# automl/CARL

Hardware: AMD Instinct MI355X
Metric: env-steps/sec (whole node) at 65k parallel contexts, 1/2/4/8 MI355X (higher is better)
Workload: dtype f32

## Files before the change

carl_amd/csrc/carl_policy.hip:

```cpp
#include <hip/hip_runtime.h>

#include <cstdint>

#include "../../include/carl_amd.h"
#include "classic_control.hip.h"
#include "host_common.hpp"
#include "policy_host.hpp"
#include "policy_kernels.hip.h"

namespace carl_host {

int policy_set_floats(const carl_policy_t* p) {
  if (p->n_in < 1 || p->n_in > CARL_POLICY_MAX_IN || p->n_out < 1 || p->n_out > 4 || p->n_hidden < 0 ||
      p->n_hidden > CARL_POLICY_MAX_HIDDEN)
    return -1;
  int64_t total = 0, prev = p->n_in;
  for (int l = 0; l <= p->n_hidden; ++l) {
    const int64_t w = l < p->n_hidden ? p->width[l] : p->n_out;
    if (l < p->n_hidden && (w < 1 || w > CARL_POLICY_MAX_WIDTH)) return -1;
    total += w * prev + w;
    prev = w;
  }
  total += 2 * (int64_t)p->n_in + 1;
  return (int)((total + 3) / 4 * 4);
}

int policy_padded_hidden(const carl_policy_t* p) {
  int wmax = 0;
  for (int l = 0; l < p->n_hidden; ++l) wmax = wmax > p->width[l] ? wmax : p->width[l];
  return p->n_hidden == 0 ? 0 : wmax <= 32 ? 32 : 64;
}

namespace {

int validate_policy(const carl_batch_t* b, const carl_policy_t* p, const carl_family_info_t& fi, const char* who) {
  if (p->n_hidden < 0 || p->n_hidden > CARL_POLICY_MAX_HIDDEN)
    return fail(CARL_ERR_INVALID_ARGUMENT, "%s: n_hidden %d outside [0, %d]", who, p->n_hidden, CARL_POLICY_MAX_HIDDEN);
  for (int l = 0; l < p->n_hidden; ++l)
    if (p->width[l] < 1 || p->width[l] > CARL_POLICY_MAX_WIDTH)
      return fail(CARL_ERR_INVALID_ARGUMENT, "%s: hidden width[%d] = %d outside [1, %d]", who, l, p->width[l],
                  CARL_POLICY_MAX_WIDTH);
  if (p->n_ctx < 0 || p->n_ctx > fi.n_features)
    return fail(CARL_ERR_INVALID_ARGUMENT, "%s: n_ctx %d outside [0, F = %d]", who, p->n_ctx, fi.n_features);
  for (int k = 0; k < p->n_ctx; ++k)
    if (p->ctx_rows[k] < 0 || p->ctx_rows[k] >= fi.n_features)
      return fail(CARL_ERR_INVALID_ARGUMENT, "%s: ctx_rows[%d] = %d is not a context-table row (F = %d)", who, k,
                  p->ctx_rows[k], fi.n_features);
  if (p->n_in != p->n_ctx + fi.obs_dim)
    return fail(CARL_ERR_INVALID_ARGUMENT, "%s: n_in %d != n_ctx %d + obs_dim %d", who, p->n_in, p->n_ctx, fi.obs_dim);
  const int want_out = fi.action_is_discrete ? fi.n_actions : 1;
  if (p->n_out != want_out)
    return fail(CARL_ERR_INVALID_ARGUMENT, "%s: head width %d, the family needs %d (%s)", who, p->n_out, want_out,
                fi.action_is_discrete ? "n_actions" : "one Box value");
  if (p->head != (fi.action_is_discrete ? CARL_POLICY_HEAD_ARGMAX : CARL_POLICY_HEAD_BOX))
    return fail(CARL_ERR_INVALID_ARGUMENT, "%s: head kind %d does not match the family's action space", who, p->head);
  if (p->activation < CARL_POLICY_IDENTITY || p->activation > CARL_POLICY_RELU)
    return fail(CARL_ERR_INVALID_ARGUMENT, "%s: unknown activation %d", who, p->activation);
  if (p->n_sets < 1) return fail(CARL_ERR_INVALID_ARGUMENT, "%s: n_sets %d < 1", who, p->n_sets);
  if (p->lanes_per_set < carl::kPolicyLanes || p->lanes_per_set % carl::kPolicyLanes != 0)
    return fail(CARL_ERR_INVALID_ARGUMENT, "%s: lanes_per_set %d is not a positive multiple of %d (carl_policy_lane_quantum)",
                who, p->lanes_per_set, carl::kPolicyLanes);
  if ((int64_t)p->n_sets * p->lanes_per_set < b->n_lanes)
    return fail(CARL_ERR_INVALID_ARGUMENT, "%s: %d sets x %d lanes do not cover %d lanes", who, p->n_sets,
                p->lanes_per_set, b->n_lanes);
  if (p->params == nullptr) return fail(CARL_ERR_INVALID_ARGUMENT, "%s: params is NULL", who);
  return 0;
}

int validate_io(const carl_batch_t* b, const carl_step_io_t* io, const carl_family_info_t& fi, const char* who) {
  if (!io->action || !io->obs || !io->reward || !io->terminated || !io->truncated)
    return fail(CARL_ERR_INVALID_ARGUMENT, "%s: a required io pointer is NULL", who);
  const int want = fi.action_is_discrete ? CARL_ACTION_I32 : CARL_ACTION_F32;
  if (io->action_dtype != want)
    return fail(CARL_ERR_INVALID_ARGUMENT, "%s: the action column is %s for this family", who,
                fi.action_is_discrete ? "int32 (CARL_ACTION_I32)" : "float32 (CARL_ACTION_F32)");
  if (io->row_pitch != 0 && io->row_pitch < b->n_lanes)
    return fail(CARL_ERR_INVALID_ARGUMENT, "%s: io.row_pitch %d < n_lanes %d", who, io->row_pitch, b->n_lanes);
  if (!carl_host::staged_rows(b, io, 15))
    return fail(CARL_ERR_UNSUPPORTED, "%s: rows of %d lanes for %d lanes: the closed-loop rollout writes the staged layout "
                "only (pitch %% 16 == 0 and n_lanes %% 16 == 0 or pitch == carl_rollout_pitch(n_lanes), arrays on 16-byte "
                "boundaries)", who, io->row_pitch > 0 ? io->row_pitch : b->n_lanes, b->n_lanes);
  return 0;
}

}

int check_rollout_policy(const char* who, const carl_batch_t* batch, const carl_policy_t* policy_host,
                         const carl_step_io_t* io, int32_t n_steps, const carl_policy_summary_t* summary_out,
                         carl_family_info_t* fi) {
  if (batch == nullptr || policy_host == nullptr) return fail(CARL_ERR_INVALID_ARGUMENT, "%s: batch / policy is NULL", who);
  if (batch->family >= CARL_N_FAMILIES)
    return fail(CARL_ERR_INVALID_ARGUMENT, "%s: family %d is a Brax family -- the closed-loop rollout covers the "
                "classic-control families only", who, batch->family);
  if (int e = validate_batch(batch, who)) return e;
  if (int e = carl_family_info(batch->family, fi)) return e;
  if (int e = validate_policy(batch, policy_host, *fi, who)) return e;
  if (n_steps < 0) return fail(CARL_ERR_INVALID_ARGUMENT, "%s: n_steps %d < 0", who, n_steps);
  if (io == nullptr) {
    if (summary_out == nullptr || !summary_out->episodes || !summary_out->return_sum || !summary_out->length_sum)
      return fail(CARL_ERR_INVALID_ARGUMENT, "%s: summary mode (io NULL) needs all three summary arrays", who);
  } else {
    if (int e = validate_io(batch, io, *fi, who)) return e;
    if (summary_out != nullptr && (!summary_out->episodes || !summary_out->return_sum || !summary_out->length_sum))
      return fail(CARL_ERR_INVALID_ARGUMENT, "%s: a summary needs all three arrays", who);
  }
  if (summary_out != nullptr && !(batch->flags & CARL_FLAG_AUTORESET))
    return fail(CARL_ERR_UNSUPPORTED, "%s: a summary needs CARL_FLAG_AUTORESET (without auto-reset a finished lane "
                "reports done on every later step, and its episode would be counted on each of them)", who);
  return 0;
}

int policy_rollout_without_steps(const char* who, const carl_batch_t* batch, const carl_policy_summary_t* summary_out,
                                 void* stream) {
  if (summary_out == nullptr || batch->n_lanes == 0) return 0;
  hipStream_t s = (hipStream_t)stream;
  const size_t bytes = (size_t)batch->n_lanes * 4;
  for (void* p : {(void*)summary_out->episodes, (void*)summary_out->return_sum, (void*)summary_out->length_sum})
    if (const hipError_t e = hipMemsetAsync(p, 0, bytes, s); e != hipSuccess)
      return fail((int)e, "%s: hipMemsetAsync: %s", who, hipGetErrorString(e));
  return 0;
}

int check_evaluate_policy(const char* who, const carl_batch_t* batch, const carl_policy_t* policy_host,
                          int32_t n_episodes, int32_t max_steps, const carl_policy_episodes_t* out,
                          carl_family_info_t* fi) {
  if (batch == nullptr || policy_host == nullptr)
    return fail(CARL_ERR_INVALID_ARGUMENT, "%s: batch / policy is NULL", who);
  if (batch->family >= CARL_N_FAMILIES)
    return fail(CARL_ERR_INVALID_ARGUMENT, "%s: family %d is a Brax family -- the closed-loop rollout covers the "
                "classic-control families only", who, batch->family);
  if (int e = validate_batch(batch, who)) return e;
  if (int e = carl_family_info(batch->family, fi)) return e;
  if (int e = validate_policy(batch, policy_host, *fi, who)) return e;
  if (out == nullptr || !out->episodes || !out->steps || !out->ret || !out->length || !out->context_id ||
      !out->terminated)
    return fail(CARL_ERR_INVALID_ARGUMENT, "%s: out and all six of its arrays are required", who);
  if (n_episodes < 1) return fail(CARL_ERR_INVALID_ARGUMENT, "%s: n_episodes %d < 1", who, n_episodes);
  if (max_steps < 0) return fail(CARL_ERR_INVALID_ARGUMENT, "%s: max_steps %d < 0", who, max_steps);
  if ((int64_t)n_episodes * batch->n_lanes >= ((int64_t)1 << 31))
    return fail(CARL_ERR_INVALID_ARGUMENT, "%s: n_episodes %d x %d lanes records do not fit 2^31 - 1", who, n_episodes,
                batch->n_lanes);
  if (!(batch->flags & CARL_FLAG_AUTORESET))
    return fail(CARL_ERR_UNSUPPORTED, "%s: needs CARL_FLAG_AUTORESET (without auto-reset a finished lane reports done on "
                "every later step, and its episode would be counted on each of them)", who);
  return 0;
}

}

namespace {

using carl_host::check_launch;
using carl_host::fail;

struct PolicyKernel {
  void (*fn)(carl_batch_t, carl_step_io_t, carl_policy_t, int, carl_policy_summary_t, int);
  size_t lds;
};

template <class Fam, int H>
PolicyKernel policy_kernel(bool summary) {
  if (summary) return {carl::policy_rollout_kernel<Fam, H, true>, carl::policy_lds_bytes<Fam, H, true>()};
  return {carl::policy_rollout_kernel<Fam, H, false>, carl::policy_lds_bytes<Fam, H, false>()};
}

template <class Fam>
int launch_policy(const carl_batch_t* b, const carl_policy_t* p, const carl_step_io_t* io, int n_steps,
                  const carl_policy_summary_t* sum, hipStream_t s) {
  const bool summary = io == nullptr;
  const int H = carl_host::policy_padded_hidden(p);
  const PolicyKernel k = H == 0 ? policy_kernel<Fam, 0>(summary) : H == 32 ? policy_kernel<Fam, 32>(summary)
                                                                  : policy_kernel<Fam, 64>(summary);
  static_assert(carl::policy_lds_bytes<Fam, 64, false>() + carl::static_lds_bytes<Fam>() <= carl::kCuLdsBytes,
                "the closed-loop rollout's LDS does not fit a compute unit");
  if (int e = carl_host::ensure_dynamic_lds(reinterpret_cast<const void*>(k.fn), k.lds, "carl_rollout_policy")) return e;
  carl_step_io_t io_r{};
  if (!summary) {
    io_r = *io;
    io_r.row_pitch = io->row_pitch > 0 ? io->row_pitch : b->n_lanes;
  }
  const carl_policy_summary_t sum_r = sum != nullptr ? *sum : carl_policy_summary_t{nullptr, nullptr, nullptr};
  const int grid = (b->n_lanes + carl::kPolicyLanes - 1) / carl::kPolicyLanes;
  const int threads = summary ? carl::kPolicyThreadsSummary : carl::kPolicyThreadsTransitions;
  hipLaunchKernelGGL(k.fn, dim3(grid), dim3(threads), k.lds, s, *b, io_r, *p, carl_host::policy_set_floats(p), sum_r, n_steps);
  return check_launch("carl_rollout_policy");
}

struct EpisodesKernel {
  void (*fn)(carl_batch_t, carl_policy_t, int, carl_policy_episodes_t, int, int);
  size_t lds;
};

template <class Fam, int H>
EpisodesKernel episodes_kernel() {
  return {carl::policy_episodes_kernel<Fam, H>, carl::policy_lds_bytes<Fam, H, true>()};
}

template <class Fam>
int launch_episodes(const carl_batch_t* b, const carl_policy_t* p, int n_episodes, int max_steps,
                    const carl_policy_episodes_t* out, hipStream_t s) {
  const int H = carl_host::policy_padded_hidden(p);
  const EpisodesKernel k = H == 0 ? episodes_kernel<Fam, 0>() : H == 32 ? episodes_kernel<Fam, 32>()
                                                               : episodes_kernel<Fam, 64>();
  if (int e = carl_host::ensure_dynamic_lds(reinterpret_cast<const void*>(k.fn), k.lds, "carl_evaluate_policy")) return e;
  const int grid = (b->n_lanes + carl::kPolicyLanes - 1) / carl::kPolicyLanes;
  hipLaunchKernelGGL(k.fn, dim3(grid), dim3(carl::kPolicyThreadsSummary), k.lds, s, *b, *p, carl_host::policy_set_floats(p), *out,
                     n_episodes, max_steps);
  return check_launch("carl_evaluate_policy");
}

}

extern "C" {

int32_t carl_policy_lane_quantum(void) { return carl::kPolicyLanes; }

int32_t carl_policy_set_floats(const carl_policy_t* policy_host) {
  if (policy_host == nullptr) return -1;
  return carl_host::policy_set_floats(policy_host);
}

int carl_rollout_policy(const carl_batch_t* batch, const carl_policy_t* policy_host, const carl_step_io_t* io,
                        int32_t n_steps, const carl_policy_summary_t* summary_out, void* stream) {
  const char* who = "carl_rollout_policy";
  carl_family_info_t fi;
  if (int e = carl_host::check_rollout_policy(who, batch, policy_host, io, n_steps, summary_out, &fi)) return e;
  if (batch->n_lanes == 0 || n_steps == 0) return carl_host::policy_rollout_without_steps(who, batch, summary_out, stream);
  return carl_host::with_classic_family(batch, [&](auto fam) {
    return launch_policy<decltype(fam)>(batch, policy_host, io, n_steps, summary_out, (hipStream_t)stream);
  });
}

int carl_evaluate_policy(const carl_batch_t* batch, const carl_policy_t* policy_host, int32_t n_episodes,
                         int32_t max_steps, const carl_policy_episodes_t* out, void* stream) {
  carl_family_info_t fi;
  if (int e = carl_host::check_evaluate_policy("carl_evaluate_policy", batch, policy_host, n_episodes, max_steps, out, &fi))
    return e;
  if (batch->n_lanes == 0) return 0;
  return carl_host::with_classic_family(batch, [&](auto fam) {
    return launch_episodes<decltype(fam)>(batch, policy_host, n_episodes, max_steps, out, (hipStream_t)stream);
  });
}

}
```

carl_amd/csrc/carl_policy_sample.hip:

```cpp
#include <hip/hip_runtime.h>

#include <cstdint>

#include "../../include/carl_amd.h"
#include "classic_control.hip.h"
#include "host_common.hpp"
#include "policy_host.hpp"
#include "policy_kernels.hip.h"

namespace {

using carl_host::check_launch;
using carl_host::fail;

int check_sampling(const char* who, const carl_policy_sampling_t* smp, const carl_family_info_t& fi, bool log_prob_ok) {
  if (smp == nullptr) return fail(CARL_ERR_INVALID_ARGUMENT, "%s: sampling is NULL", who);
  if (!fi.action_is_discrete && smp->log_std == nullptr)
    return fail(CARL_ERR_INVALID_ARGUMENT, "%s: a Box family needs sampling->log_std ([n_sets] on the device)", who);
  if (!log_prob_ok && smp->log_prob != nullptr)
    return fail(CARL_ERR_INVALID_ARGUMENT, "%s: sampling->log_prob is a transitions-mode output (io != NULL); this mode "
                "stores nothing per step", who);
  if ((reinterpret_cast<uintptr_t>(smp->log_prob) & 15) != 0)
    return fail(CARL_ERR_UNSUPPORTED, "%s: sampling->log_prob is not on a 16-byte boundary", who);
  return 0;
}

struct SampledKernel {
  void (*fn)(carl_batch_t, carl_step_io_t, carl_policy_t, int, carl_policy_summary_t, int, carl_policy_sampling_t);
  size_t lds;
};

template <class Fam, int H>
SampledKernel sampled_kernel(bool summary, bool logp) {
  using carl::policy_lds_bytes;
  if (summary) return {carl::policy_rollout_sampled_kernel<Fam, H, true, false>, policy_lds_bytes<Fam, H, true>()};
  if (logp) return {carl::policy_rollout_sampled_kernel<Fam, H, false, true>, policy_lds_bytes<Fam, H, false, true>()};
  return {carl::policy_rollout_sampled_kernel<Fam, H, false, false>, policy_lds_bytes<Fam, H, false>()};
}

template <class Fam>
int launch_sampled(const carl_batch_t* b, const carl_policy_t* p, const carl_policy_sampling_t* smp,
                   const carl_step_io_t* io, int n_steps, const carl_policy_summary_t* sum, hipStream_t s) {
  const bool summary = io == nullptr, logp = smp->log_prob != nullptr;
  const int H = carl_host::policy_padded_hidden(p);
  const SampledKernel k = H == 0 ? sampled_kernel<Fam, 0>(summary, logp) : H == 32 ? sampled_kernel<Fam, 32>(summary, logp)
                                                                          : sampled_kernel<Fam, 64>(summary, logp);
  static_assert(carl::policy_lds_bytes<Fam, 64, false, true>() + carl::static_lds_bytes<Fam>() <= carl::kCuLdsBytes,
                "the sampled rollout's LDS (the log_prob column included) does not fit a compute unit");
  if (int e = carl_host::ensure_dynamic_lds(reinterpret_cast<const void*>(k.fn), k.lds, "carl_rollout_policy_sampled"))
    return e;
  carl_step_io_t io_r{};
  if (!summary) {
    io_r = *io;
    io_r.row_pitch = io->row_pitch > 0 ? io->row_pitch : b->n_lanes;
  }
  const carl_policy_summary_t sum_r = sum != nullptr ? *sum : carl_policy_summary_t{nullptr, nullptr, nullptr};
  const int grid = (b->n_lanes + carl::kPolicyLanes - 1) / carl::kPolicyLanes;
  const int threads = summary ? carl::kPolicyThreadsSummary : carl::kPolicyThreadsTransitions;
  hipLaunchKernelGGL(k.fn, dim3(grid), dim3(threads), k.lds, s, *b, io_r, *p, carl_host::policy_set_floats(p), sum_r,
                     n_steps, *smp);
  return check_launch("carl_rollout_policy_sampled");
}

struct SampledEpisodesKernel {
  void (*fn)(carl_batch_t, carl_policy_t, int, carl_policy_episodes_t, int, int, carl_policy_sampling_t);
  size_t lds;
};

template <class Fam, int H>
SampledEpisodesKernel sampled_episodes_kernel() {
  return {carl::policy_episodes_sampled_kernel<Fam, H>, carl::policy_lds_bytes<Fam, H, true>()};
}

template <class Fam>
int launch_sampled_episodes(const carl_batch_t* b, const carl_policy_t* p, const carl_policy_sampling_t* smp,
                            int n_episodes, int max_steps, const carl_policy_episodes_t* out, hipStream_t s) {
  const int H = carl_host::policy_padded_hidden(p);
  const SampledEpisodesKernel k = H == 0 ? sampled_episodes_kernel<Fam, 0>() : H == 32 ? sampled_episodes_kernel<Fam, 32>()
                                                                              : sampled_episodes_kernel<Fam, 64>();
  if (int e = carl_host::ensure_dynamic_lds(reinterpret_cast<const void*>(k.fn), k.lds, "carl_evaluate_policy_sampled"))
    return e;
  const int grid = (b->n_lanes + carl::kPolicyLanes - 1) / carl::kPolicyLanes;
  hipLaunchKernelGGL(k.fn, dim3(grid), dim3(carl::kPolicyThreadsSummary), k.lds, s, *b, *p,
                     carl_host::policy_set_floats(p), *out, n_episodes, max_steps, *smp);
  return check_launch("carl_evaluate_policy_sampled");
}

}

extern "C" {

int carl_rollout_policy_sampled(const carl_batch_t* batch, const carl_policy_t* policy_host,
                                const carl_policy_sampling_t* sampling, const carl_step_io_t* io, int32_t n_steps,
                                const carl_policy_summary_t* summary_out, void* stream) {
  const char* who = "carl_rollout_policy_sampled";
  carl_family_info_t fi;
  if (int e = carl_host::check_rollout_policy(who, batch, policy_host, io, n_steps, summary_out, &fi)) return e;
  if (int e = check_sampling(who, sampling, fi, io != nullptr)) return e;
  if (batch->n_lanes == 0 || n_steps == 0) return carl_host::policy_rollout_without_steps(who, batch, summary_out, stream);
  return carl_host::with_classic_family(batch, [&](auto fam) {
    return launch_sampled<decltype(fam)>(batch, policy_host, sampling, io, n_steps, summary_out, (hipStream_t)stream);
  });
}

int carl_evaluate_policy_sampled(const carl_batch_t* batch, const carl_policy_t* policy_host,
                                 const carl_policy_sampling_t* sampling, int32_t n_episodes, int32_t max_steps,
                                 const carl_policy_episodes_t* out, void* stream) {
  const char* who = "carl_evaluate_policy_sampled";
  carl_family_info_t fi;
  if (int e = carl_host::check_evaluate_policy(who, batch, policy_host, n_episodes, max_steps, out, &fi)) return e;
  if (int e = check_sampling(who, sampling, fi, false)) return e;
  if (batch->n_lanes == 0) return 0;
  return carl_host::with_classic_family(batch, [&](auto fam) {
    return launch_sampled_episodes<decltype(fam)>(batch, policy_host, sampling, n_episodes, max_steps, out,
                                                  (hipStream_t)stream);
  });
}

}
```

carl_amd/csrc/policy_episodes_body.inc:

```
  using L = PolicyLayout<Fam, H>;
  using Action = typename Fam::Action;
  constexpr int CHUNK = policy_chunk<Fam>();
  extern __shared__ float lds_dyn[];
  stage_family_tables<Fam>();
  float* const wts = lds_dyn;
  const int lane_base = (int)blockIdx.x * kPolicyLanes;
  stage_policy<Fam, H>(wts, pol, set_floats, lane_base / pol.lanes_per_set);
  const GlobalCtx ctx{b.ctx_table, b.ctx_stride};
  const int lane = lane_base + (int)threadIdx.x;
  const bool active = lane < b.n_lanes;
  const uint64_t glane = (uint64_t)(b.lane_offset + lane);
  const size_t n = (size_t)b.n_lanes;
  __syncthreads();

  LaneRegs<Fam> r{};
  load_staged_lane<Fam>(b, ctx, lane, active, r);
  const int n_ctx = pol.n_ctx, n_hidden = pol.n_hidden, act = pol.activation;
  const int w0 = pol.width[0], w1 = pol.width[1];
  const float clip = wts[L::kClip];
  float x[L::K];
#pragma unroll
  for (int s = 0; s < L::K; ++s) x[s] = 0.0f;
  int x_cidx = -1;
  int done_eps = 0, steps = 0;
  bool live = active;
  for (int t0 = 0; t0 < max_steps && ballot(live) != 0ull; t0 += CHUNK) {
    if constexpr (predraw_of<Fam>::value) predraw<Fam>(b, glane, r);
    const int n_u = min(CHUNK, max_steps - t0);
#pragma unroll 1
    for (int u = 0; u < n_u; ++u) {
      if (ballot(live) == 0ull) break;
      if (ballot(r.cidx != x_cidx) != 0ull) {
#pragma unroll
        for (int k = 0; k < Fam::F; ++k)
          if (k < n_ctx) x[k] = normalize_input(ctx.get(pol.ctx_rows[k], r.cidx), wts[L::kShift + k], wts[L::kScale + k], clip);
        x_cidx = r.cidx;
      }
      float o[Fam::D];
      Fam::observe(r.s, r.aux, o);
#pragma unroll
      for (int d = 0; d < Fam::D; ++d)
        x[Fam::F + d] = normalize_input(o[d], wts[L::kShift + Fam::F + d], wts[L::kScale + Fam::F + d], clip);
      [[maybe_unused]] float lp;
      Action a;
      if constexpr (Pick::kSampled)
        a = pick.template choose<H>(wts, x, n_hidden, act, w0, w1, glane, r, lp);
      else
        a = policy_action<Fam, H>(wts, x, n_hidden, act, w0, w1);
      const int before = r.n_new_episodes, cidx = r.cidx;
      bool te = false;
      step_lane<Fam, GlobalCtx, false, TermSink<Fam>>(b, ctx, TermSink<Fam>{&te}, b.max_episode_steps, live, lane,
                                                       glane, a, r);
      steps += live ? 1 : 0;
      if (r.n_new_episodes != before) {
        const size_t at = (size_t)done_eps * n + lane;
        ep.ret[at] = r.fin_return;
        ep.length[at] = r.fin_length;
        ep.context_id[at] = cidx;
        ep.terminated[at] = (uint8_t)te;
        done_eps += 1;
      }
      live = live && done_eps < n_episodes;
    }
  }
  if (active) {
    store_lane<Fam>(b, ctx, lane, r);
    ep.episodes[lane] = done_eps;
    ep.steps[lane] = steps;
    for (int k = done_eps; k < n_episodes; ++k) {
      const size_t at = (size_t)k * n + lane;
      ep.ret[at] = __builtin_nanf("");
      ep.length[at] = 0;
      ep.context_id[at] = -1;
      ep.terminated[at] = 0;
    }
  }
```

carl_amd/csrc/policy_host.hpp:

```cpp
#pragma once

#include <cstdint>

#include "../../include/carl_amd.h"

namespace carl_host {
int policy_set_floats(const carl_policy_t* p);
int policy_padded_hidden(const carl_policy_t* p);

int check_rollout_policy(const char* who, const carl_batch_t* batch, const carl_policy_t* policy, const carl_step_io_t* io,
                         int32_t n_steps, const carl_policy_summary_t* summary_out, carl_family_info_t* fi);
int check_evaluate_policy(const char* who, const carl_batch_t* batch, const carl_policy_t* policy, int32_t n_episodes,
                          int32_t max_steps, const carl_policy_episodes_t* out, carl_family_info_t* fi);
int policy_rollout_without_steps(const char* who, const carl_batch_t* batch, const carl_policy_summary_t* summary_out,
                                 void* stream);
}
```

carl_amd/csrc/policy_kernels.hip.h:

```cpp
#pragma once

#include "engine_kernels.hip.h"

namespace carl {

constexpr int kPolicyLanes = kRolloutLanes;
constexpr int kPolicyThreadsSummary = kPolicyLanes;
constexpr int kPolicyThreadsTransitions = kPolicyLanes + kStorers * kWave;

template <class Fam>
struct policy_outputs : std::integral_constant<int, std::is_same_v<typename Fam::Action, float> ? 1
                                                    : (std::is_same_v<Fam, CartPole> ? 2 : 3)> {};

template <class Fam, int H>
struct PolicyLayout {
  static constexpr int K = (Fam::F + Fam::D + 3) / 4 * 4;
  static constexpr int HI = H == 0 ? K : H;
  static constexpr int kW1 = 0, kB1 = kW1 + H * K, kW2 = kB1 + H, kB2 = kW2 + H * H, kWh = kB2 + H, kBh = kWh + HI * 4;
  static constexpr int kShift = kBh + 4, kScale = kShift + K, kClip = kScale + K;
  static constexpr int kFloats = kClip + 4;
  static constexpr size_t kBytes = (size_t)kFloats * sizeof(float);
};

template <bool LOGP>
__host__ __device__ constexpr size_t policy_logp_lds_bytes(int chunk) {
  return LOGP ? (size_t)2 * chunk * kPolicyLanes * 4 : 0;
}
template <class Fam, bool LOGP = false>
__host__ __device__ constexpr int policy_chunk() {
  return rollout_staged_lds_bytes<Fam, 8>() + policy_logp_lds_bytes<LOGP>(8) + PolicyLayout<Fam, 64>::kBytes +
                     static_lds_bytes<Fam>() <= kCuLdsBytes ? 8 : 4;
}
template <class Fam, int H, bool SUMMARY, bool LOGP = false>
__host__ __device__ constexpr size_t policy_lds_bytes() {
  constexpr int CHUNK = policy_chunk<Fam, LOGP>();
  return PolicyLayout<Fam, H>::kBytes +
         (SUMMARY ? 0 : rollout_staged_lds_bytes<Fam, CHUNK>() + policy_logp_lds_bytes<LOGP>(CHUNK));
}

template <class Fam, int H>
__device__ __forceinline__ void stage_policy(float* w, const carl_policy_t& pol, int set_floats, int set) {
  using L = PolicyLayout<Fam, H>;
  const float* src = pol.params + (size_t)set * set_floats;
  const int n_in = pol.n_in, n_ctx = pol.n_ctx, n_out = pol.n_out;
  const int nh = pol.n_hidden;
  const int w0 = nh > 0 ? pol.width[0] : 0, w1 = nh > 1 ? pol.width[1] : 0;
  const int dims[CARL_POLICY_MAX_HIDDEN + 2] = {n_in, nh > 0 ? w0 : n_out, nh > 1 ? w1 : n_out, n_out};
  int p_w[CARL_POLICY_MAX_HIDDEN + 1] = {0, 0, 0}, p_b[CARL_POLICY_MAX_HIDDEN + 1] = {0, 0, 0};
  int off = 0;
#pragma unroll
  for (int l = 0; l <= CARL_POLICY_MAX_HIDDEN; ++l) {
    if (l <= nh) {
      p_w[l] = off;
      off += dims[l + 1] * dims[l];
      p_b[l] = off;
      off += dims[l + 1];
    }
  }
  const int p_w0 = p_w[0], p_b0 = p_b[0], p_w1 = p_w[1], p_b1 = p_b[1];
  const int p_shift = off, p_scale = p_shift + n_in, p_clip = p_scale + n_in;
  auto in_of = [&](int s) -> int {
    if (s < n_ctx) return s;
    if (s >= Fam::F && s < Fam::F + Fam::D) return n_ctx + (s - Fam::F);
    return -1;
  };
  const int hw = p_w[nh], hb = p_b[nh], hin = dims[nh];
  for (int e = threadIdx.x; e < L::kFloats; e += blockDim.x) {
    float v = 0.0f;
    if (e < L::kB1) {
      const int j = e / L::K, s = e % L::K, i = in_of(s);
      if (j < w0 && i >= 0) v = src[p_w0 + j * n_in + i];
    } else if (e < L::kW2) {
      const int j = e - L::kB1;
      if (j < w0) v = src[p_b0 + j];
    } else if (e < L::kB2) {
      const int j = (e - L::kW2) / (H > 0 ? H : 1), i = (e - L::kW2) % (H > 0 ? H : 1);
      if (j < w1 && i < w0) v = src[p_w1 + j * w0 + i];
    } else if (e < L::kWh) {
      const int j = e - L::kB2;
      if (j < w1) v = src[p_b1 + j];
    } else if (e < L::kBh) {
      const int j = (e - L::kWh) / 4, k = (e - L::kWh) % 4;
      const int i = H == 0 ? in_of(j) : (j < hin ? j : -1);
      if (k < n_out && i >= 0) v = src[hw + k * hin + i];
    } else if (e < L::kShift) {
      const int k = e - L::kBh;
      if (k < n_out) v = src[hb + k];
    } else if (e < L::kScale) {
      const int i = in_of(e - L::kShift);
      if (i >= 0) v = src[p_shift + i];
    } else if (e < L::kClip) {
      const int i = in_of(e - L::kScale);
      if (i >= 0) v = src[p_scale + i];
    } else {
      v = src[p_clip];
    }
    w[e] = v;
  }
}

typedef float pvf4 __attribute__((ext_vector_type(4)));

__device__ __forceinline__ pvf4 bcast4(const float* p) { return *reinterpret_cast<const pvf4*>(p); }

__device__ __forceinline__ float tanh_fast(float v) {
#pragma clang fp contract(off)
  const float e = __expf(2.0f * v);
  return 1.0f - __fdividef(2.0f, e + 1.0f);
}

template <int N>
__device__ __forceinline__ void activate(float (&h)[N], int act, int width) {
  if (act == CARL_POLICY_TANH) {
#pragma unroll
    for (int j = 0; j < N; ++j) h[j] = tanh_fast(h[j]);
  } else if (act == CARL_POLICY_RELU) {
#pragma unroll
    for (int j = 0; j < N; ++j) h[j] = fmaxf(h[j], 0.0f);
  }
  if (width < N) {
#pragma unroll
    for (int j = 0; j < N; ++j) h[j] = j < width ? h[j] : 0.0f;
  }
}

template <int OUT, int IN>
__device__ __forceinline__ void dense_layer(const float* w, const float* b, const float (&in)[IN], float (&out)[OUT]) {
  static_assert(IN % 4 == 0 && OUT % 4 == 0, "LDS rows are read as float4");
#pragma unroll
  for (int j0 = 0; j0 < OUT; j0 += 4) {
    const pvf4 bb = bcast4(b + j0);
    float acc[4] = {bb.x, bb.y, bb.z, bb.w};
#pragma unroll
    for (int i = 0; i < IN; i += 4) {
#pragma unroll
      for (int jj = 0; jj < 4; ++jj) {
        const pvf4 ww = bcast4(w + (j0 + jj) * IN + i);
        acc[jj] = __fmaf_rn(ww.x, in[i], acc[jj]);
        acc[jj] = __fmaf_rn(ww.y, in[i + 1], acc[jj]);
        acc[jj] = __fmaf_rn(ww.z, in[i + 2], acc[jj]);
        acc[jj] = __fmaf_rn(ww.w, in[i + 3], acc[jj]);
      }
    }
#pragma unroll
    for (int jj = 0; jj < 4; ++jj) out[j0 + jj] = acc[jj];
  }
}

template <int IN>
__device__ __forceinline__ void head_layer(const float* wt, const float* b, const float (&in)[IN], float (&y)[4]) {
  const pvf4 bb = bcast4(b);
  y[0] = bb.x, y[1] = bb.y, y[2] = bb.z, y[3] = bb.w;
#pragma unroll
  for (int j = 0; j < IN; ++j) {
    const pvf4 ww = bcast4(wt + 4 * j);
    y[0] = __fmaf_rn(ww.x, in[j], y[0]);
    y[1] = __fmaf_rn(ww.y, in[j], y[1]);
    y[2] = __fmaf_rn(ww.z, in[j], y[2]);
    y[3] = __fmaf_rn(ww.w, in[j], y[3]);
  }
}

__device__ __forceinline__ float normalize_input(float v, float shift, float scale, float clip) {
#pragma clang fp contract(off)
  return fminf(fmaxf((v - shift) * scale, -clip), clip);
}

template <class Fam, int H>
__device__ __forceinline__ void policy_head(const float* w, const float (&x)[PolicyLayout<Fam, H>::K], int n_hidden,
                                            int act, int w0, int w1, float (&y)[4]) {
  using L = PolicyLayout<Fam, H>;
  if constexpr (H == 0) {
    head_layer<L::K>(w + L::kWh, w + L::kBh, x, y);
  } else {
    float h1[H];
    dense_layer<H, L::K>(w + L::kW1, w + L::kB1, x, h1);
    activate(h1, act, w0);
    if (n_hidden > 1) {
      float h2[H];
      dense_layer<H, H>(w + L::kW2, w + L::kB2, h1, h2);
      activate(h2, act, w1);
      head_layer<H>(w + L::kWh, w + L::kBh, h2, y);
    } else {
      head_layer<H>(w + L::kWh, w + L::kBh, h1, y);
    }
  }
}

template <class Fam, int H>
__device__ __forceinline__ typename Fam::Action policy_action(const float* w, const float (&x)[PolicyLayout<Fam, H>::K],
                                                              int n_hidden, int act, int w0, int w1) {
  using L = PolicyLayout<Fam, H>;
  float y[4];
  if constexpr (H == 0) {
    head_layer<L::K>(w + L::kWh, w + L::kBh, x, y);
  } else {
    float h1[H];
    dense_layer<H, L::K>(w + L::kW1, w + L::kB1, x, h1);
    activate(h1, act, w0);
    if (n_hidden > 1) {
      float h2[H];
      dense_layer<H, H>(w + L::kW2, w + L::kB2, h1, h2);
      activate(h2, act, w1);
      head_layer<H>(w + L::kWh, w + L::kBh, h2, y);
    } else {
      head_layer<H>(w + L::kWh, w + L::kBh, h1, y);
    }
  }
  if constexpr (std::is_same_v<typename Fam::Action, float>) {
    return y[0];
  } else {
    int best = 0;
    float top = y[0];
#pragma unroll
    for (int k = 1; k < policy_outputs<Fam>::value; ++k) {
      const bool gt = y[k] > top;
      best = gt ? k : best;
      top = gt ? y[k] : top;
    }
    return best;
  }
}

template <class Fam>
struct ModePick {
  static constexpr bool kSampled = false, kLogProb = false;
};

template <class Fam, bool LOGP>
struct SampledPick {
  static constexpr bool kSampled = true, kLogProb = LOGP;
  uint64_t seed;
  float sigma;
  float lp0;

  static __device__ __forceinline__ SampledPick of(const carl_policy_sampling_t& smp, const carl_policy_t& pol) {
    SampledPick p{smp.seed, 1.0f, 0.0f};
    if constexpr (std::is_same_v<typename Fam::Action, float>) {
      const float ls = smp.log_std[(int)blockIdx.x * kPolicyLanes / pol.lanes_per_set];
      p.sigma = expf(ls);
      p.lp0 = -ls - 0.918938533204672742f;
    }
    return p;
  }

  template <int H>
  __device__ __forceinline__ typename Fam::Action choose(const float* w, const float (&x)[PolicyLayout<Fam, H>::K],
                                                         int n_hidden, int act, int w0, int w1, uint64_t glane,
                                                         const LaneRegs<Fam>& r, float& lp) const {
#pragma clang fp contract(off)
    const u32x4 wd = lane_words(seed, glane, r.episode - 1u, kSubSample | (uint32_t)r.elapsed);
    float y[4];
    if constexpr (std::is_same_v<typename Fam::Action, float>) {
      const float u1 = (float)((wd.x >> 8) + 1u) * (1.0f / 16777216.0f);
      const float u2 = u01(wd.y);
      const float z = sqrtf(-2.0f * logf(u1)) * cospif(2.0f * u2);
      policy_head<Fam, H>(w, x, n_hidden, act, w0, w1, y);
      if constexpr (LOGP) lp = __fmaf_rn(-0.5f * z, z, lp0);
      return __fmaf_rn(sigma, z, y[0]);
    } else {
      constexpr int NA = policy_outputs<Fam>::value;
      const float u = u01(wd.x);
      policy_head<Fam, H>(w, x, n_hidden, act, w0, w1, y);
      float m = y[0];
#pragma unroll
      for (int k = 1; k < NA; ++k) m = fmaxf(m, y[k]);
      float c[NA];
      float s = 0.0f;
#pragma unroll
      for (int k = 0; k < NA; ++k) c[k] = s = s + expf(y[k] - m);
      const float t = u * s;
      int a = NA - 1;
      float ya = y[NA - 1];
#pragma unroll
      for (int k = NA - 2; k >= 0; --k) {
        const bool in = t < c[k];
        a = in ? k : a;
        ya = in ? y[k] : ya;
      }
      if constexpr (LOGP) lp = (ya - m) - logf(s);
      return a;
    }
  }
};

template <class Fam>
struct NullSink {
  static constexpr bool kLazyFlags = true;
  __device__ __forceinline__ void put_reward(float) const {}
  __device__ __forceinline__ void put_flags(bool, bool) const {}
  __device__ __forceinline__ void put_obs(const float (&)[Fam::D]) const {}
  __device__ __forceinline__ float* final_obs_ptr() const { return nullptr; }
};

__device__ __forceinline__ void drain_actions(const char* buf, void* action, size_t n, int cols, int lane_base, int l,
                                              int which, int t0, int steps) {
  const int valid = min(kPolicyLanes, cols - lane_base);
  for (int u = which; u < steps; u += kStorers) {
    const char* src = buf + (size_t)u * kPolicyLanes * 4 + 16 * l;
    char* dst = reinterpret_cast<char*>(action) + ((size_t)(t0 + u) * n + lane_base) * 4 + 16 * l;
    if (4 * l < valid) __builtin_nontemporal_store(*reinterpret_cast<const pvf4*>(src), reinterpret_cast<pvf4*>(dst));
  }
}

template <class Fam, int H, bool SUMMARY>
__global__ void __launch_bounds__(SUMMARY ? kPolicyThreadsSummary : kPolicyThreadsTransitions)
    policy_rollout_kernel(const carl_batch_t b, const carl_step_io_t io, const carl_policy_t pol, const int set_floats,
                          const carl_policy_summary_t sum, const int n_steps) {
  using Pick = ModePick<Fam>;
  const Pick pick{};
  float* const log_prob = nullptr;
#include "policy_rollout_body.inc"
}

template <class Fam, int H, bool SUMMARY, bool LOGP>
__global__ void __launch_bounds__(SUMMARY ? kPolicyThreadsSummary : kPolicyThreadsTransitions)
    policy_rollout_sampled_kernel(const carl_batch_t b, const carl_step_io_t io, const carl_policy_t pol,
                                  const int set_floats, const carl_policy_summary_t sum, const int n_steps,
                                  const carl_policy_sampling_t smp) {
  static_assert(!(SUMMARY && LOGP), "a summary stores no per-step column");
  using Pick = SampledPick<Fam, LOGP>;
  const Pick pick = Pick::of(smp, pol);
  float* const log_prob = smp.log_prob;
#include "policy_rollout_body.inc"
}

template <class Fam>
struct TermSink {
  static constexpr bool kLazyFlags = true;
  bool* te;
  __device__ __forceinline__ void put_reward(float) const {}
  __device__ __forceinline__ void put_flags(bool t, bool) const { *te = t; }
  __device__ __forceinline__ void put_obs(const float (&)[Fam::D]) const {}
  __device__ __forceinline__ float* final_obs_ptr() const { return nullptr; }
};

template <class Fam, int H>
__global__ void __launch_bounds__(kPolicyThreadsSummary)
    policy_episodes_kernel(const carl_batch_t b, const carl_policy_t pol, const int set_floats,
                           const carl_policy_episodes_t ep, const int n_episodes, const int max_steps) {
  using Pick = ModePick<Fam>;
  const Pick pick{};
#include "policy_episodes_body.inc"
}

template <class Fam, int H>
__global__ void __launch_bounds__(kPolicyThreadsSummary)
    policy_episodes_sampled_kernel(const carl_batch_t b, const carl_policy_t pol, const int set_floats,
                                   const carl_policy_episodes_t ep, const int n_episodes, const int max_steps,
                                   const carl_policy_sampling_t smp) {
  using Pick = SampledPick<Fam, false>;
  const Pick pick = Pick::of(smp, pol);
#include "policy_episodes_body.inc"
}

}
```

carl_amd/csrc/policy_rollout_body.inc:

```
  using L = PolicyLayout<Fam, H>;
  using SK = LdsSink<Fam>;
  using Action = typename Fam::Action;
  constexpr int CHUNK = policy_chunk<Fam, Pick::kLogProb>();
  extern __shared__ float lds_dyn[];
  stage_family_tables<Fam>();
  float* const wts = lds_dyn;
  char* const out_buf = reinterpret_cast<char*>(lds_dyn) + L::kBytes;
  char* const act_buf = out_buf + (size_t)2 * CHUNK * SK::kStepBytes;
  char* const lp_buf = act_buf + (size_t)2 * CHUNK * kPolicyLanes * 4;
  const int lane_base = (int)blockIdx.x * kPolicyLanes;
  stage_policy<Fam, H>(wts, pol, set_floats, lane_base / pol.lanes_per_set);
  const GlobalCtx ctx{b.ctx_table, b.ctx_stride};
  const int wave = __builtin_amdgcn_readfirstlane((int)(threadIdx.x / kWave));
  const bool compute = wave < kPolicyLanes / kWave;
  const int hl = threadIdx.x % kWave;
  const int storer = wave - kPolicyLanes / kWave;
  const int lane = lane_base + (compute ? (int)threadIdx.x : 0);
  const bool active = compute && lane < b.n_lanes;
  const uint64_t glane = (uint64_t)(b.lane_offset + lane);
  const size_t n = (size_t)io.row_pitch;
  const int n_cols = (b.n_lanes + 15) & ~15;
  if (!SUMMARY && !compute) zero_flag_rows<Fam, CHUNK>(out_buf, hl, storer);
  __syncthreads();

  if (compute) {
    LaneRegs<Fam> r{};
    load_staged_lane<Fam>(b, ctx, lane, active, r);
    float* const final_base = (!SUMMARY && io.final_obs != nullptr && active) ? io.final_obs + (size_t)lane * Fam::D : nullptr;
    const int n_ctx = pol.n_ctx, n_hidden = pol.n_hidden, act = pol.activation;
    const int w0 = pol.width[0], w1 = pol.width[1];
    const float clip = wts[L::kClip];
    float x[L::K];
#pragma unroll
    for (int s = 0; s < L::K; ++s) x[s] = 0.0f;
    int x_cidx = -1;
    int ep_count = 0, len_sum = 0;
    float ret_sum = 0.0f;
    int buf = 0;
    for (int t0 = 0; t0 < n_steps; t0 += CHUNK, buf ^= 1) {
      const int steps = min(CHUNK, n_steps - t0);
      if constexpr (predraw_of<Fam>::value) predraw<Fam>(b, glane, r);
      char* const rec = out_buf + (size_t)buf * CHUNK * SK::kStepBytes;
      Action* const my_act = reinterpret_cast<Action*>(act_buf + (size_t)buf * CHUNK * kPolicyLanes * 4) + threadIdx.x;
#pragma unroll 1
      for (int u = 0; u < steps; ++u) {
        if (ballot(r.cidx != x_cidx) != 0ull) {
#pragma unroll
          for (int k = 0; k < Fam::F; ++k)
            if (k < n_ctx) x[k] = normalize_input(ctx.get(pol.ctx_rows[k], r.cidx), wts[L::kShift + k], wts[L::kScale + k], clip);
          x_cidx = r.cidx;
        }
        float o[Fam::D];
        Fam::observe(r.s, r.aux, o);
#pragma unroll
        for (int d = 0; d < Fam::D; ++d)
          x[Fam::F + d] = normalize_input(o[d], wts[L::kShift + Fam::F + d], wts[L::kScale + Fam::F + d], clip);
        [[maybe_unused]] float lp;
        Action a;
        if constexpr (Pick::kSampled)
          a = pick.template choose<H>(wts, x, n_hidden, act, w0, w1, glane, r, lp);
        else
          a = policy_action<Fam, H>(wts, x, n_hidden, act, w0, w1);
        const int before = r.n_new_episodes;
        if constexpr (SUMMARY) {
          step_lane<Fam, GlobalCtx, true, NullSink<Fam>>(b, ctx, NullSink<Fam>{}, b.max_episode_steps, true, lane, glane,
                                                          a, r);
        } else {
          my_act[u * kPolicyLanes] = a;
          if constexpr (Pick::kLogProb)
            reinterpret_cast<float*>(lp_buf + (size_t)buf * CHUNK * kPolicyLanes * 4)[u * kPolicyLanes + threadIdx.x] = lp;
          const SK sink{rec + (size_t)u * SK::kStepBytes, final_base, n * Fam::D, t0 + u, (int)threadIdx.x};
          step_lane<Fam, GlobalCtx, true, SK>(b, ctx, sink, b.max_episode_steps, true, lane, glane, a, r);
        }
        const bool fin = r.n_new_episodes != before;
        ep_count += fin ? 1 : 0;
        len_sum += fin ? r.fin_length : 0;
        ret_sum = fin ? ret_sum + r.fin_return : ret_sum;
      }
      if constexpr (!SUMMARY) __syncthreads();
    }
    if (active) {
      store_lane<Fam>(b, ctx, lane, r);
      if (sum.episodes != nullptr) {
        sum.episodes[lane] = ep_count;
        sum.return_sum[lane] = ret_sum;
        sum.length_sum[lane] = len_sum;
      }
    }
  } else if constexpr (!SUMMARY) {
    int buf = 0;
    for (int t0 = 0; t0 < n_steps; t0 += CHUNK, buf ^= 1) {
      if (t0 > 0) {
        drain_records<Fam>(out_buf + (size_t)(buf ^ 1) * CHUNK * SK::kStepBytes, io, n, n_cols, lane_base, hl, storer,
                           t0 - CHUNK, CHUNK);
        drain_actions(act_buf + (size_t)(buf ^ 1) * CHUNK * kPolicyLanes * 4, const_cast<void*>(io.action), n, n_cols,
                      lane_base, hl, storer, t0 - CHUNK, CHUNK);
        if constexpr (Pick::kLogProb)
          drain_actions(lp_buf + (size_t)(buf ^ 1) * CHUNK * kPolicyLanes * 4, log_prob, n, n_cols, lane_base, hl,
                        storer, t0 - CHUNK, CHUNK);
      }
      __syncthreads();
    }
    if (n_steps > 0) {
      const int last_t0 = ((n_steps - 1) / CHUNK) * CHUNK;
      drain_records<Fam>(out_buf + (size_t)(buf ^ 1) * CHUNK * SK::kStepBytes, io, n, n_cols, lane_base, hl, storer,
                         last_t0, n_steps - last_t0);
      drain_actions(act_buf + (size_t)(buf ^ 1) * CHUNK * kPolicyLanes * 4, const_cast<void*>(io.action), n, n_cols,
                    lane_base, hl, storer, last_t0, n_steps - last_t0);
      if constexpr (Pick::kLogProb)
        drain_actions(lp_buf + (size_t)(buf ^ 1) * CHUNK * kPolicyLanes * 4, log_prob, n, n_cols, lane_base, hl, storer,
                      last_t0, n_steps - last_t0);
    }
  }
```

Before: 211.4 billion.

## Serve hidden-layer policy weights through scalar loads from a padded global copy

For hidden-layer policies, the weights are no longer staged into LDS per block. A small pre-kernel pads each weight set into a scratch buffer allocated with hipMallocAsync, and the rollout and episode kernels read it through constant-address-space (scalar) loads. New dense and head layer routines software-pipeline these loads with explicit waitcnt and sched barriers. This frees LDS, which can allow larger step chunks and more blocks per CU, at the cost of an extra launch plus an alloc and free on every call, and scalar-cache pressure.

Measured after the change: 211.2 billion, median of 4. Within noise of the previous version (-0.1%).

```diff
diff --git a/carl_amd/csrc/carl_policy.hip b/carl_amd/csrc/carl_policy.hip
--- a/carl_amd/csrc/carl_policy.hip
+++ b/carl_amd/csrc/carl_policy.hip
@@ -146,6 +146,50 @@
   return 0;
 }
 
+namespace {
+
+template <class Fam>
+int pad_policy(const carl_policy_t* p, int H, int sets, float* dst, hipStream_t s) {
+  const int packed = policy_set_floats(p);
+  if (H == 32)
+    hipLaunchKernelGGL((carl::pad_policy_kernel<Fam, 32>), dim3(sets), dim3(carl::kPolicyLanes), 0, s, *p, packed, dst);
+  else
+    hipLaunchKernelGGL((carl::pad_policy_kernel<Fam, 64>), dim3(sets), dim3(carl::kPolicyLanes), 0, s, *p, packed, dst);
+  return H == 32 ? carl::PolicyLayout<Fam, 32>::kFloats : carl::PolicyLayout<Fam, 64>::kFloats;
+}
+
+}
+
+int feed_policy(const char* who, const carl_batch_t* b, const carl_policy_t* p, void* stream, PolicyFeed* feed) {
+  *feed = {*p, policy_set_floats(p), nullptr};
+  const int H = policy_padded_hidden(p);
+  if (H == 0) return 0;
+  hipStream_t s = (hipStream_t)stream;
+  const int used = (b->n_lanes + p->lanes_per_set - 1) / p->lanes_per_set;
+  const int sets = used < p->n_sets ? used : p->n_sets;
+  const size_t bytes = (size_t)sets * 32 * 1024;
+  if (const hipError_t e = hipMallocAsync(reinterpret_cast<void**>(&feed->scratch), bytes, s); e != hipSuccess)
+    return fail((int)e, "%s: hipMallocAsync of %zu bytes for the padded weight sets: %s", who, bytes, hipGetErrorString(e));
+  feed->pol.params = feed->scratch;
+  feed->set_floats = with_classic_family(b, [&](auto fam) {
+    using Fam = decltype(fam);
+    static_assert(carl::PolicyLayout<Fam, 64>::kBytes <= 32 * 1024, "a padded weight set does not fit its slot");
+    return pad_policy<Fam>(p, H, sets, feed->scratch, s);
+  });
+  if (int e = check_launch(who)) {
+    (void)hipFreeAsync(feed->scratch, s);
+    return e;
+  }
+  return 0;
+}
+
+int release_feed(const char* who, const PolicyFeed& feed, void* stream) {
+  if (feed.scratch == nullptr) return 0;
+  if (const hipError_t e = hipFreeAsync(feed.scratch, (hipStream_t)stream); e != hipSuccess)
+    return fail((int)e, "%s: hipFreeAsync: %s", who, hipGetErrorString(e));
+  return 0;
+}
+
 }
 
 namespace {
@@ -182,8 +226,12 @@
   const carl_policy_summary_t sum_r = sum != nullptr ? *sum : carl_policy_summary_t{nullptr, nullptr, nullptr};
   const int grid = (b->n_lanes + carl::kPolicyLanes - 1) / carl::kPolicyLanes;
   const int threads = summary ? carl::kPolicyThreadsSummary : carl::kPolicyThreadsTransitions;
-  hipLaunchKernelGGL(k.fn, dim3(grid), dim3(threads), k.lds, s, *b, io_r, *p, carl_host::policy_set_floats(p), sum_r, n_steps);
-  return check_launch("carl_rollout_policy");
+  carl_host::PolicyFeed feed;
+  if (int e = carl_host::feed_policy("carl_rollout_policy", b, p, s, &feed)) return e;
+  hipLaunchKernelGGL(k.fn, dim3(grid), dim3(threads), k.lds, s, *b, io_r, feed.pol, feed.set_floats, sum_r, n_steps);
+  const int e = check_launch("carl_rollout_policy");
+  const int e_free = carl_host::release_feed("carl_rollout_policy", feed, s);
+  return e != 0 ? e : e_free;
 }
 
 struct EpisodesKernel {
@@ -204,9 +252,13 @@
                                                                : episodes_kernel<Fam, 64>();
   if (int e = carl_host::ensure_dynamic_lds(reinterpret_cast<const void*>(k.fn), k.lds, "carl_evaluate_policy")) return e;
   const int grid = (b->n_lanes + carl::kPolicyLanes - 1) / carl::kPolicyLanes;
-  hipLaunchKernelGGL(k.fn, dim3(grid), dim3(carl::kPolicyThreadsSummary), k.lds, s, *b, *p, carl_host::policy_set_floats(p), *out,
+  carl_host::PolicyFeed feed;
+  if (int e = carl_host::feed_policy("carl_evaluate_policy", b, p, s, &feed)) return e;
+  hipLaunchKernelGGL(k.fn, dim3(grid), dim3(carl::kPolicyThreadsSummary), k.lds, s, *b, feed.pol, feed.set_floats, *out,
                      n_episodes, max_steps);
-  return check_launch("carl_evaluate_policy");
+  const int e = check_launch("carl_evaluate_policy");
+  const int e_free = carl_host::release_feed("carl_evaluate_policy", feed, s);
+  return e != 0 ? e : e_free;
 }
 
 }
diff --git a/carl_amd/csrc/carl_policy_sample.hip b/carl_amd/csrc/carl_policy_sample.hip
--- a/carl_amd/csrc/carl_policy_sample.hip
+++ b/carl_amd/csrc/carl_policy_sample.hip
@@ -57,9 +57,12 @@
   const carl_policy_summary_t sum_r = sum != nullptr ? *sum : carl_policy_summary_t{nullptr, nullptr, nullptr};
   const int grid = (b->n_lanes + carl::kPolicyLanes - 1) / carl::kPolicyLanes;
   const int threads = summary ? carl::kPolicyThreadsSummary : carl::kPolicyThreadsTransitions;
-  hipLaunchKernelGGL(k.fn, dim3(grid), dim3(threads), k.lds, s, *b, io_r, *p, carl_host::policy_set_floats(p), sum_r,
-                     n_steps, *smp);
-  return check_launch("carl_rollout_policy_sampled");
+  carl_host::PolicyFeed feed;
+  if (int e = carl_host::feed_policy("carl_rollout_policy_sampled", b, p, s, &feed)) return e;
+  hipLaunchKernelGGL(k.fn, dim3(grid), dim3(threads), k.lds, s, *b, io_r, feed.pol, feed.set_floats, sum_r, n_steps, *smp);
+  const int e = check_launch("carl_rollout_policy_sampled");
+  const int e_free = carl_host::release_feed("carl_rollout_policy_sampled", feed, s);
+  return e != 0 ? e : e_free;
 }
 
 struct SampledEpisodesKernel {
@@ -81,9 +84,13 @@
   if (int e = carl_host::ensure_dynamic_lds(reinterpret_cast<const void*>(k.fn), k.lds, "carl_evaluate_policy_sampled"))
     return e;
   const int grid = (b->n_lanes + carl::kPolicyLanes - 1) / carl::kPolicyLanes;
-  hipLaunchKernelGGL(k.fn, dim3(grid), dim3(carl::kPolicyThreadsSummary), k.lds, s, *b, *p,
-                     carl_host::policy_set_floats(p), *out, n_episodes, max_steps, *smp);
-  return check_launch("carl_evaluate_policy_sampled");
+  carl_host::PolicyFeed feed;
+  if (int e = carl_host::feed_policy("carl_evaluate_policy_sampled", b, p, s, &feed)) return e;
+  hipLaunchKernelGGL(k.fn, dim3(grid), dim3(carl::kPolicyThreadsSummary), k.lds, s, *b, feed.pol, feed.set_floats, *out,
+                     n_episodes, max_steps, *smp);
+  const int e = check_launch("carl_evaluate_policy_sampled");
+  const int e_free = carl_host::release_feed("carl_evaluate_policy_sampled", feed, s);
+  return e != 0 ? e : e_free;
 }
 
 }
diff --git a/carl_amd/csrc/policy_episodes_body.inc b/carl_amd/csrc/policy_episodes_body.inc
--- a/carl_amd/csrc/policy_episodes_body.inc
+++ b/carl_amd/csrc/policy_episodes_body.inc
@@ -3,9 +3,8 @@
   constexpr int CHUNK = policy_chunk<Fam>();
   extern __shared__ float lds_dyn[];
   stage_family_tables<Fam>();
-  float* const wts = lds_dyn;
   const int lane_base = (int)blockIdx.x * kPolicyLanes;
-  stage_policy<Fam, H>(wts, pol, set_floats, lane_base / pol.lanes_per_set);
+  const policy_wptr<H> wts0 = policy_weights<Fam, H>(lds_dyn, pol, set_floats, lane_base / pol.lanes_per_set);
   const GlobalCtx ctx{b.ctx_table, b.ctx_stride};
   const int lane = lane_base + (int)threadIdx.x;
   const bool active = lane < b.n_lanes;
@@ -17,7 +16,7 @@
   load_staged_lane<Fam>(b, ctx, lane, active, r);
   const int n_ctx = pol.n_ctx, n_hidden = pol.n_hidden, act = pol.activation;
   const int w0 = pol.width[0], w1 = pol.width[1];
-  const float clip = wts[L::kClip];
+  const float clip = wts0[L::kClip];
   float x[L::K];
 #pragma unroll
   for (int s = 0; s < L::K; ++s) x[s] = 0.0f;
@@ -30,6 +29,7 @@
 #pragma unroll 1
     for (int u = 0; u < n_u; ++u) {
       if (ballot(live) == 0ull) break;
+      const policy_wptr<H> wts = per_step(wts0);
       if (ballot(r.cidx != x_cidx) != 0ull) {
 #pragma unroll
         for (int k = 0; k < Fam::F; ++k)
diff --git a/carl_amd/csrc/policy_host.hpp b/carl_amd/csrc/policy_host.hpp
--- a/carl_amd/csrc/policy_host.hpp
+++ b/carl_amd/csrc/policy_host.hpp
@@ -14,4 +14,12 @@
                           int32_t max_steps, const carl_policy_episodes_t* out, carl_family_info_t* fi);
 int policy_rollout_without_steps(const char* who, const carl_batch_t* batch, const carl_policy_summary_t* summary_out,
                                  void* stream);
+
+struct PolicyFeed {
+  carl_policy_t pol;
+  int set_floats;
+  float* scratch;
+};
+int feed_policy(const char* who, const carl_batch_t* batch, const carl_policy_t* p, void* stream, PolicyFeed* feed);
+int release_feed(const char* who, const PolicyFeed& feed, void* stream);
 }
diff --git a/carl_amd/csrc/policy_kernels.hip.h b/carl_amd/csrc/policy_kernels.hip.h
--- a/carl_amd/csrc/policy_kernels.hip.h
+++ b/carl_amd/csrc/policy_kernels.hip.h
@@ -26,15 +26,19 @@
 __host__ __device__ constexpr size_t policy_logp_lds_bytes(int chunk) {
   return LOGP ? (size_t)2 * chunk * kPolicyLanes * 4 : 0;
 }
+template <class Fam, int H>
+__host__ __device__ constexpr size_t policy_weight_lds_bytes() {
+  return H == 0 ? PolicyLayout<Fam, 0>::kBytes : 0;
+}
 template <class Fam, bool LOGP = false>
 __host__ __device__ constexpr int policy_chunk() {
-  return rollout_staged_lds_bytes<Fam, 8>() + policy_logp_lds_bytes<LOGP>(8) + PolicyLayout<Fam, 64>::kBytes +
+  return rollout_staged_lds_bytes<Fam, 8>() + policy_logp_lds_bytes<LOGP>(8) + policy_weight_lds_bytes<Fam, 0>() +
                      static_lds_bytes<Fam>() <= kCuLdsBytes ? 8 : 4;
 }
 template <class Fam, int H, bool SUMMARY, bool LOGP = false>
 __host__ __device__ constexpr size_t policy_lds_bytes() {
   constexpr int CHUNK = policy_chunk<Fam, LOGP>();
-  return PolicyLayout<Fam, H>::kBytes +
+  return policy_weight_lds_bytes<Fam, H>() +
          (SUMMARY ? 0 : rollout_staged_lds_bytes<Fam, CHUNK>() + policy_logp_lds_bytes<LOGP>(CHUNK));
 }
 
@@ -100,8 +104,37 @@
 }
 
 typedef float pvf4 __attribute__((ext_vector_type(4)));
+typedef float pvf8 __attribute__((ext_vector_type(8), aligned(16)));
+
+typedef const float __attribute__((address_space(4))) * policy_sptr;
+template <int H>
+using policy_wptr = std::conditional_t<H == 0, const float*, policy_sptr>;
 
 __device__ __forceinline__ pvf4 bcast4(const float* p) { return *reinterpret_cast<const pvf4*>(p); }
+template <class V>
+__device__ __forceinline__ V sload(policy_sptr p) {
+  return *reinterpret_cast<const V __attribute__((address_space(4)))*>(p);
+}
+__device__ __forceinline__ void block_arrived(policy_sptr& w, policy_sptr& b, float (&acc)[4]) {
+  __builtin_amdgcn_s_waitcnt(0xc07f);
+  asm volatile("" : "+s"(w), "+s"(b), "+v"(acc[0]), "+v"(acc[1]), "+v"(acc[2]), "+v"(acc[3]));
+}
+
+template <class Fam, int H>
+__device__ __forceinline__ policy_wptr<H> policy_weights(float* lds, const carl_policy_t& pol, int set_floats, int set) {
+  if constexpr (H == 0) {
+    stage_policy<Fam, 0>(lds, pol, set_floats, set);
+    return lds;
+  } else {
+    return (policy_sptr)(uintptr_t)(pol.params + (size_t)set * set_floats);
+  }
+}
+
+__device__ __forceinline__ const float* per_step(const float* w) { return w; }
+__device__ __forceinline__ policy_sptr per_step(policy_sptr w) {
+  asm volatile("" : "+s"(w));
+  return w;
+}
 
 __device__ __forceinline__ float tanh_fast(float v) {
 #pragma clang fp contract(off)
@@ -147,6 +180,44 @@
   }
 }
 
+template <int OUT, int IN>
+__device__ __forceinline__ void dense_layer(policy_sptr w, policy_sptr b, const float (&in)[IN], float (&out)[OUT]) {
+  static_assert(IN % 4 == 0 && OUT % 4 == 0, "rows are read as float4 / float8");
+  constexpr int CH = IN % 8 == 0 ? 8 : 4, NI = IN / CH, NB = OUT / 4 * NI;
+  using V = std::conditional_t<CH == 8, pvf8, pvf4>;
+  V cur[4], nxt[4];
+  pvf4 bias;
+  float acc[4];
+#pragma unroll
+  for (int jj = 0; jj < 4; ++jj) cur[jj] = sload<V>(w + jj * IN);
+  bias = sload<pvf4>(b);
+#pragma unroll
+  for (int blk = 0; blk < NB; ++blk) {
+    const int j0 = blk / NI * 4, i = blk % NI * CH;
+    if (i == 0) acc[0] = bias.x, acc[1] = bias.y, acc[2] = bias.z, acc[3] = bias.w;
+    block_arrived(w, b, acc);
+    if (blk + 1 < NB) {
+      const int j1 = (blk + 1) / NI * 4, i1 = (blk + 1) % NI * CH;
+#pragma unroll
+      for (int jj = 0; jj < 4; ++jj) nxt[jj] = sload<V>(w + (j1 + jj) * IN + i1);
+      if (i1 == 0) bias = sload<pvf4>(b + j1);
+    }
+    __builtin_amdgcn_sched_barrier(0);
+#pragma unroll
+    for (int k = 0; k < CH; ++k) {
+#pragma unroll
+      for (int jj = 0; jj < 4; ++jj) acc[jj] = __fmaf_rn(cur[jj][k], in[i + k], acc[jj]);
+    }
+    __builtin_amdgcn_sched_barrier(0);
+    if (i + CH == IN) {
+#pragma unroll
+      for (int jj = 0; jj < 4; ++jj) out[j0 + jj] = acc[jj];
+    }
+#pragma unroll
+    for (int jj = 0; jj < 4; ++jj) cur[jj] = nxt[jj];
+  }
+}
+
 template <int IN>
 __device__ __forceinline__ void head_layer(const float* wt, const float* b, const float (&in)[IN], float (&y)[4]) {
   const pvf4 bb = bcast4(b);
@@ -161,13 +232,41 @@
   }
 }
 
+template <int IN>
+__device__ __forceinline__ void head_layer(policy_sptr wt, policy_sptr b, const float (&in)[IN], float (&y)[4]) {
+  static_assert(IN % 8 == 0, "the hidden widths are multiples of 8");
+  constexpr int NB = IN / 8;
+  pvf8 cur[4], nxt[4];
+#pragma unroll
+  for (int q = 0; q < 4; ++q) cur[q] = sload<pvf8>(wt + 8 * q);
+  const pvf4 bb = sload<pvf4>(b);
+#pragma unroll
+  for (int blk = 0; blk < NB; ++blk) {
+    if (blk == 0) y[0] = bb.x, y[1] = bb.y, y[2] = bb.z, y[3] = bb.w;
+    block_arrived(wt, b, y);
+    if (blk + 1 < NB) {
+#pragma unroll
+      for (int q = 0; q < 4; ++q) nxt[q] = sload<pvf8>(wt + 32 * (blk + 1) + 8 * q);
+    }
+    __builtin_amdgcn_sched_barrier(0);
+#pragma unroll
+    for (int jj = 0; jj < 8; ++jj) {
+#pragma unroll
+      for (int k = 0; k < 4; ++k) y[k] = __fmaf_rn(cur[jj / 2][4 * (jj % 2) + k], in[8 * blk + jj], y[k]);
+    }
+    __builtin_amdgcn_sched_barrier(0);
+#pragma unroll
+    for (int q = 0; q < 4; ++q) cur[q] = nxt[q];
+  }
+}
+
 __device__ __forceinline__ float normalize_input(float v, float shift, float scale, float clip) {
 #pragma clang fp contract(off)
   return fminf(fmaxf((v - shift) * scale, -clip), clip);
 }
 
 template <class Fam, int H>
-__device__ __forceinline__ void policy_head(const float* w, const float (&x)[PolicyLayout<Fam, H>::K], int n_hidden,
+__device__ __forceinline__ void policy_head(policy_wptr<H> w, const float (&x)[PolicyLayout<Fam, H>::K], int n_hidden,
                                             int act, int w0, int w1, float (&y)[4]) {
   using L = PolicyLayout<Fam, H>;
   if constexpr (H == 0) {
@@ -188,7 +287,7 @@
 }
 
 template <class Fam, int H>
-__device__ __forceinline__ typename Fam::Action policy_action(const float* w, const float (&x)[PolicyLayout<Fam, H>::K],
+__device__ __forceinline__ typename Fam::Action policy_action(policy_wptr<H> w, const float (&x)[PolicyLayout<Fam, H>::K],
                                                               int n_hidden, int act, int w0, int w1) {
   using L = PolicyLayout<Fam, H>;
   float y[4];
@@ -245,7 +344,7 @@
   }
 
   template <int H>
-  __device__ __forceinline__ typename Fam::Action choose(const float* w, const float (&x)[PolicyLayout<Fam, H>::K],
+  __device__ __forceinline__ typename Fam::Action choose(policy_wptr<H> w, const float (&x)[PolicyLayout<Fam, H>::K],
                                                          int n_hidden, int act, int w0, int w1, uint64_t glane,
                                                          const LaneRegs<Fam>& r, float& lp) const {
 #pragma clang fp contract(off)
@@ -303,6 +402,12 @@
   }
 }
 
+template <class Fam, int H>
+__global__ void __launch_bounds__(kPolicyLanes)
+    pad_policy_kernel(const carl_policy_t pol, const int set_floats, float* const dst) {
+  stage_policy<Fam, H>(dst + (size_t)blockIdx.x * PolicyLayout<Fam, H>::kFloats, pol, set_floats, (int)blockIdx.x);
+}
+
 template <class Fam, int H, bool SUMMARY>
 __global__ void __launch_bounds__(SUMMARY ? kPolicyThreadsSummary : kPolicyThreadsTransitions)
     policy_rollout_kernel(const carl_batch_t b, const carl_step_io_t io, const carl_policy_t pol, const int set_floats,
diff --git a/carl_amd/csrc/policy_rollout_body.inc b/carl_amd/csrc/policy_rollout_body.inc
--- a/carl_amd/csrc/policy_rollout_body.inc
+++ b/carl_amd/csrc/policy_rollout_body.inc
@@ -4,12 +4,11 @@
   constexpr int CHUNK = policy_chunk<Fam, Pick::kLogProb>();
   extern __shared__ float lds_dyn[];
   stage_family_tables<Fam>();
-  float* const wts = lds_dyn;
-  char* const out_buf = reinterpret_cast<char*>(lds_dyn) + L::kBytes;
+  char* const out_buf = reinterpret_cast<char*>(lds_dyn) + policy_weight_lds_bytes<Fam, H>();
   char* const act_buf = out_buf + (size_t)2 * CHUNK * SK::kStepBytes;
   char* const lp_buf = act_buf + (size_t)2 * CHUNK * kPolicyLanes * 4;
   const int lane_base = (int)blockIdx.x * kPolicyLanes;
-  stage_policy<Fam, H>(wts, pol, set_floats, lane_base / pol.lanes_per_set);
+  const policy_wptr<H> wts0 = policy_weights<Fam, H>(lds_dyn, pol, set_floats, lane_base / pol.lanes_per_set);
   const GlobalCtx ctx{b.ctx_table, b.ctx_stride};
   const int wave = __builtin_amdgcn_readfirstlane((int)(threadIdx.x / kWave));
   const bool compute = wave < kPolicyLanes / kWave;
@@ -29,7 +28,7 @@
     float* const final_base = (!SUMMARY && io.final_obs != nullptr && active) ? io.final_obs + (size_t)lane * Fam::D : nullptr;
     const int n_ctx = pol.n_ctx, n_hidden = pol.n_hidden, act = pol.activation;
     const int w0 = pol.width[0], w1 = pol.width[1];
-    const float clip = wts[L::kClip];
+    const float clip = wts0[L::kClip];
     float x[L::K];
 #pragma unroll
     for (int s = 0; s < L::K; ++s) x[s] = 0.0f;
@@ -44,6 +43,7 @@
       Action* const my_act = reinterpret_cast<Action*>(act_buf + (size_t)buf * CHUNK * kPolicyLanes * 4) + threadIdx.x;
 #pragma unroll 1
       for (int u = 0; u < steps; ++u) {
+        const policy_wptr<H> wts = per_step(wts0);
         if (ballot(r.cidx != x_cidx) != 0ull) {
 #pragma unroll
           for (int k = 0; k < Fam::F; ++k)
```
